# hedgepigdaniel/video-annotator

Hardware: AMD Instinct MI355X
Metric: stabilized frames/sec at 4K NV12, 1/2/4/8 GPU; remap % HBM roofline (higher is better)
Workload: dtype u8 pixels / f32 map / f64 rotations

## Files before the change

### video-annotator_amd/csrc/vstab_testhooks.cpp

```cpp
#include <algorithm>

#include "vstab_detect_host.hpp"
#include "vstab_hostlogic.hpp"
#include "vstab_pipeline.hpp"
#include "vstab_track_host.hpp"
#include "vstab_warp_bands.hpp"
#include "vstab_warp_request.hpp"

using namespace vstab;

extern "C" {
__attribute__((visibility("default"))) int vstabx_parse_records(const uint32_t *rec, int n, uint32_t seq, int expect_n, float *xy, unsigned char *status,
                                                                 int *n_out, int *next) {
    std::vector<float> pts;
    std::vector<uint8_t> st;
    int nx = 0;
    const LkParse r = lk_parse_records(rec, 0, n, seq, (size_t)expect_n, pts, st, &nx);
    for (size_t i = 0; i < st.size(); i++) xy[2 * i] = pts[2 * i], xy[2 * i + 1] = pts[2 * i + 1], status[i] = st[i];
    *n_out = (int)st.size(), *next = nx;
    return (int)r;
}
__attribute__((visibility("default"))) int vstabx_dmabuf_cache_sim(const unsigned long long *ids, const size_t *sizes, int n, int cap, long window,
                                                                    long long fail_id, long *counts, unsigned long long *bases) {
    DmaBufCache<unsigned long long> cache;
// ... 176 lines not shown
                                                                       double k, int block, int response, unsigned int cap, unsigned int canary,
                                                                       unsigned long long *keys_out, unsigned int *counts_out, unsigned int *tile_counts,
                                                                       int *max_bits_out, void *stream) {
    if (response != VSTAB_CORNER_MIN_EIGENVAL && response != VSTAB_CORNER_HARRIS) return fail(VSTAB_ERR_INVALID, "vstabx_corners_fused_block: response is 0 or 1");
    return corners_fused_hook("vstabx_corners_fused_block", gray, pitch, w, h, mask, pitch_mask, mask != nullptr, quality, cap, canary, keys_out, counts_out, tile_counts,
                              stream, response == VSTAB_CORNER_HARRIS, k, max_bits_out, block);
}
__attribute__((visibility("default"))) int vstabx_corners_fused_grad(const void *gray, size_t pitch, int w, int h, const void *mask, size_t pitch_mask, double quality,
                                                                      double k, int block, int gradient, int response, unsigned int cap, unsigned int canary,
                                                                      unsigned long long *keys_out, unsigned int *counts_out, unsigned int *tile_counts,
                                                                      int *max_bits_out, void *stream) {
    if (response != VSTAB_CORNER_MIN_EIGENVAL && response != VSTAB_CORNER_HARRIS) return fail(VSTAB_ERR_INVALID, "vstabx_corners_fused_grad: response is 0 or 1");
    return corners_fused_hook("vstabx_corners_fused_grad", gray, pitch, w, h, mask, pitch_mask, mask != nullptr, quality, cap, canary, keys_out, counts_out, tile_counts,
                              stream, response == VSTAB_CORNER_HARRIS, k, max_bits_out, block, gradient);
}

__attribute__((visibility("default"))) int vstabx_weighted_bands(int dw, int dh, int rwb, int lds_kb, double tail_rounds, const uint32_t *cost, int n_cost,
                                                                  int *out) {
    if (!out || dw < 1 || dh < 1 || (rwb != 4 && rwb != 8) || lds_kb < 1 || !(tail_rounds >= 0.0) || n_cost < 0)
        return fail(VSTAB_ERR_INVALID, "vstabx_weighted_bands: bad argument");
    FusedArgs ta = {};
    ta.w.dw = dw, ta.w.dh = dh;
    const unsigned grid = cost ? weighted_bands(ta, rwb, lds_kb, tail_rounds, cost, n_cost) : tile_schedule(ta, rwb, lds_kb, tail_rounds);
    for (int k = 0; k < 9; k++) out[k] = ta.band_y[k];
    for (int k = 0; k < 8; k++) out[9 + k] = ta.split_y[k];
    out[17] = ta.tiles_x, out[18] = (int)grid;
    return VSTAB_OK;
}
__attribute__((visibility("default"))) int vstabx_band_costs(const float *params, int nan_behind, int sw, int sh, int dw, int dh, int ts, uint32_t *cost, int n_cost) {
    if (!params || !cost || sw < 1 || sh < 1 || dw < 1 || dh < 1 || (ts != 8 && ts != 16) || n_cost != (int)div_up((unsigned)dh, (unsigned)ts))
        return fail(VSTAB_ERR_INVALID, "vstabx_band_costs: bad argument");
    std::vector<uint32_t> c;
    band_costs(params, nan_behind != 0, sw, sh, dw, dh, ts, c);
    std::copy(c.begin(), c.end(), cost);
    return VSTAB_OK;
}
__attribute__((visibility("default"))) int vstabx_band_cache_run(const float *params, int n, int sw, int sh, int dw, int dh, int map_mode, int rwb, int lds_kb,
                                                                  double tail_rounds, int *out, long *counts) {
    if (!params || !out || !counts || n < 1 || sw < 1 || sh < 1 || dw < 1 || dh < 1 || (rwb != 4 && rwb != 8) || lds_kb < 1 || !(tail_rounds >= 0.0))
        return fail(VSTAB_ERR_INVALID, "vstabx_band_cache_run: bad argument");
    BandCache cache;
    for (int i = 0; i < n; i++) {
        FusedArgs ta = {};
        ta.w.sw = sw, ta.w.sh = sh, ta.w.dw = dw, ta.w.dh = dh;
        const unsigned grid = cache.schedule(ta, params + 17 * (size_t)i, map_mode, rwb, lds_kb, tail_rounds);
        int *o = out + 19 * (size_t)i;
        for (int k = 0; k < 9; k++) o[k] = ta.band_y[k];
        for (int k = 0; k < 8; k++) o[9 + k] = ta.split_y[k];
        o[17] = ta.tiles_x, o[18] = (int)grid;
    }
    counts[0] = cache.hits, counts[1] = cache.misses, counts[2] = (long)cache.entries.size();
    return VSTAB_OK;
}

__attribute__((visibility("default"))) int vstabx_warp_route(int map_mode, int lens, int rs, int resample, int border_entry, int border_mode, int out_format, int keep,
                                                              int qmap, int *out) {
    if (!out) return fail(VSTAB_ERR_INVALID, "vstabx_warp_route: bad argument");
    const WarpRoute r = warp_route(map_mode, lens, rs != 0, resample, border_entry, border_mode, out_format, keep != 0, qmap != 0);
    out[0] = r.family, out[1] = r.block, out[2] = r.mode;
    return VSTAB_OK;
}

__attribute__((visibility("default"))) int vstabx_select_corners(const unsigned long long *keys, unsigned int n, int w, int h, int max_corners, double min_distance,
                                                                  float *xy, int *count) {
    if ((n > 0 && !keys) || !xy || !count || w < 1 || h < 1 || !(min_distance >= 0.0))
        return fail(VSTAB_ERR_INVALID, "vstabx_select_corners: bad argument");
    for (unsigned int i = 0; i < n; i++)
        if ((keys[i] & 0xffffffffu) >= (uint64_t)w * (uint64_t)h) return fail(VSTAB_ERR_INVALID, "vstabx_select_corners: a key names a pixel outside the image");
    std::vector<unsigned long long> k(keys, keys + n);
    std::vector<float> out;
    select_corners(k.data(), n, w, h, max_corners, min_distance, out);
    std::copy(out.begin(), out.end(), xy);
    *count = (int)(out.size() / 2);
    return VSTAB_OK;
}

__attribute__((visibility("default"))) int vstabx_detector_counters(const vstab_handle *h, long *out) {
    if (!h || !out) return fail(VSTAB_ERR_INVALID, "vstabx_detector_counters: bad argument");
    out[0] = h->detector.spec_over_cap(), out[1] = h->detector.fused_overflows(), out[2] = (long)h->detector.key_capacity();
    return VSTAB_OK;
}

__attribute__((visibility("default"))) int vstabx_pack_pyr(const void *y, size_t pitch_y, const void *uv, size_t pitch_uv, int w, int h, void *ring, void *dst,
                                                            size_t dpitch, void *stream) {
    if (!pack_pyr_ok(y, pitch_y, uv, pitch_uv, w, h, ring, dst, dpitch)) return -1;
    return launch_pack_pyr(static_cast<const uint8_t *>(y), pitch_y, static_cast<const uint8_t *>(uv), pitch_uv, w, h, static_cast<uint8_t *>(ring),
                           static_cast<uint8_t *>(dst), dpitch, static_cast<hipStream_t>(stream));
}
__attribute__((visibility("default"))) int vstabx_launch_pack_pyr(const void *y, size_t pitch_y, const void *uv, size_t pitch_uv, int w, int h, void *ring, void *dst,
                                                                   size_t dpitch, void *stream) {
    return launch_pack_pyr(static_cast<const uint8_t *>(y), pitch_y, static_cast<const uint8_t *>(uv), pitch_uv, w, h, static_cast<uint8_t *>(ring),
                           static_cast<uint8_t *>(dst), dpitch, static_cast<hipStream_t>(stream));
}
__attribute__((visibility("default"))) int vstabx_pyr_down_check(size_t pitch_src, int w, int h, size_t pitch_mid, size_t pitch_dst, int two_levels) {
    return two_levels ? check_pyr_down_x2(pitch_src, w, h, pitch_mid, pitch_dst) : check_pyr_down(pitch_src, w, h, pitch_dst);
}
}
```

### video-annotator_amd/csrc/vstab_warp_args.hpp

```cpp
#pragma once
#include "vstab_device.hpp"
#include "vstab_internal.hpp"

namespace vstab {

struct WarpArgs {
    const uint8_t *y;
    const uint8_t *uv;
    uint8_t *dst;
    uint8_t *dst_uv;
    size_t pitch_y, pitch_uv, pitch_dst, pitch_dst_uv;
    int sw, sh, dw, dh;
    MapParams p;
};

struct FusedArgs {
    WarpArgs w;
    MapParams32 p32;
    int lds_capacity_px;
    int src_vec_ok;
    int dst_vec_ok;
    int tiles_x, tiles_y;
    const int2 *qmap;
    int qpitch;
    float rs_d[9];
    float rs_den;
    int band_y[9];
    int split_y[8];
#ifdef VSTAB_DEV
    unsigned long long *timing;
    int ablate;
    int lds_pad;
#endif
    ColourCoef col;
};

template <typename K>
__device__ __forceinline__ void fetch_tap(const WarpArgs &a, const K &k, int X, int Y, int &b, int &g, int &r) {
    if ((unsigned)X < (unsigned)a.sw && (unsigned)Y < (unsigned)a.sh) {
        const int yv = a.y[(size_t)Y * a.pitch_y + X];
        const uint16_t c = *reinterpret_cast<const uint16_t *>(a.uv + (size_t)(Y >> 1) * a.pitch_uv + (X & ~1));
        yuv_to_bgr(k, yv, chroma_term(k, c & 255, c >> 8), b, g, r);
    } else {
        b = g = r = 0;
    }
}
__device__ __forceinline__ void fetch_tap(const WarpArgs &a, int X, int Y, int &b, int &g, int &r) { fetch_tap(a, CvtColor8{}, X, Y, b, g, r); }

template <typename K>
__device__ __forceinline__ uint32_t gather_pixel(const WarpArgs &a, const K &k, int sx, int sy) {
    const int X = sx >> 5, Y = sy >> 5;
    const uint32_t fx = sx & 31, fy = sy & 31;
    const int w00 = (32 - fx) * (32 - fy), w01 = fx * (32 - fy), w10 = (32 - fx) * fy, w11 = fx * fy;
    int b0, g0, r0, b1, g1, r1, b2, g2, r2, b3, g3, r3;
    fetch_tap(a, k, X, Y, b0, g0, r0);
    fetch_tap(a, k, X + 1, Y, b1, g1, r1);
    fetch_tap(a, k, X, Y + 1, b2, g2, r2);
    fetch_tap(a, k, X + 1, Y + 1, b3, g3, r3);
    const uint32_t B = (uint32_t)(b0 * w00 + b1 * w01 + b2 * w10 + b3 * w11 + 512) >> 10;
    const uint32_t G = (uint32_t)(g0 * w00 + g1 * w01 + g2 * w10 + g3 * w11 + 512) >> 10;
    const uint32_t R = (uint32_t)(r0 * w00 + r1 * w01 + r2 * w10 + r3 * w11 + 512) >> 10;
    return B | (G << 8) | (R << 16);
}

__device__ __forceinline__ uint32_t load_u32_bytes(const uint8_t *p, int valid) {
    uint32_t v = 0;
    for (int i = 0; i < 4; i++)
        if (i < valid) v |= (uint32_t)p[i] << (8 * i);
    return v;
}

vstab_status launch_warp_fused(const WarpArgs &a, const float params[17], int map_mode, bool nv12_out, bool src_vec_ok, bool dst_vec_ok,
                               const void *qmap, int qpitch, const float *rot_bottom, hipStream_t st, const float *dist = nullptr);
vstab_status launch_warp_fused_colour(const WarpArgs &a, const float params[17], int map_mode, bool nv12_out, bool src_vec_ok, bool dst_vec_ok, const ColourCoef &col,
                                      hipStream_t st);
vstab_status launch_warp_fused10(const WarpArgs &a, const float params[17], int map_mode, int blend, const float *rot_bottom, bool p010_out, bool src_vec_ok,
                                 bool dst_vec_ok, hipStream_t st, const ColourCoef *col = nullptr);

vstab_status launch_warp_planar(const WarpArgs &a, const float params[17], int map_mode, int depth, int blend, bool src_vec_ok, bool dst_vec_ok,
                                const float *rot_bottom, hipStream_t st, const float *dist = nullptr);

}
```

### video-annotator_amd/csrc/vstab_warp_bands.hpp

```cpp
#pragma once
#include <array>
#include <cmath>
#include <cstdint>
#include <cstring>
#include <mutex>
#include <vector>

#include "vstab_warp_tile.hpp"

namespace vstab {

static inline unsigned weighted_bands(FusedArgs &ta, int rwb, int lds_kb, double tail_rounds, const uint32_t *cost, int n_cost) {
    const unsigned even_grid = tile_schedule(ta, rwb, lds_kb, tail_rounds);
    const WarpArgs &a = ta.w;
    const int th = 4 * rwb, ts = th / 2;
    const int half_rows = (int)div_up(a.dh, ts);
    if (!cost || n_cost != half_rows) return even_grid;
    uint64_t total = 0;
    for (int i = 0; i < half_rows; i++) total += cost[i];
    if (total == 0) return even_grid;
    const int slots = 32 * std::max(1, std::min(8, (int)(160 / lds_kb)));
    int h = 0;
    uint64_t prefix = 0;
    ta.band_y[0] = 0;
    for (int k = 1; k < 8; k++) {
        while (h < half_rows && 8 * (prefix + cost[h]) <= (uint64_t)k * total) prefix += cost[h++];
        ta.band_y[k] = std::min(a.dh, h * ts);
    }
    ta.band_y[8] = a.dh;
    int share = 0;
    for (int k = 0; k < 8; k++) {
        const int rows = ta.band_y[k + 1] - ta.band_y[k];
        const int tall_rows_max = rows / th;
        const int tail_tall_rows = (int)std::min<long>(tall_rows_max, std::lround(tail_rounds * slots / ta.tiles_x));
        const int tall_rows = tall_rows_max - tail_tall_rows;
        ta.split_y[k] = ta.band_y[k] + tall_rows * th;
        const int n = tall_rows * ta.tiles_x + (int)div_up(ta.band_y[k + 1] - ta.split_y[k], ts) * ta.tiles_x;
        share = std::max(share, n);
    }
    return 8u * (unsigned)share;
}

constexpr uint32_t BAND_COST_DEAD = 135, BAND_COST_LIVE = 220;
constexpr double BAND_COST_PER_BLOCK = 0.45;

static inline void band_costs(const float params[17], bool nan_behind, int sw, int sh, int dw, int dh, int ts, std::vector<uint32_t> &cost) {
    const int tiles_x = (int)div_up(dw, 64), half_rows = (int)div_up(dh, ts);
    const double icx = params[0], icy = params[1], ifx = params[2], ify = params[3], ocx = params[4], ocy = params[5], ofx = params[6], ofy = params[7];
    const float *r = params + 8;
    std::vector<double> X((size_t)(tiles_x + 1) * 2), Y((size_t)(tiles_x + 1) * 2);
    auto corners = [&](int row, double *xo, double *yo) {
        const double vy = ((double)std::min(row * ts, dh - 1) - ocy) / ofy;
        for (int c = 0; c <= tiles_x; c++) {
            const double vx = ((double)std::min(c * 64, dw - 1) - ocx) / ofx;
            const double wx = r[0] * vx + r[1] * vy + r[2], wy = r[3] * vx + r[4] * vy + r[5], wz = r[6] * vx + r[7] * vy + r[8];
            if (!(wz > 0.0) && (nan_behind || wz == 0.0)) {
                xo[c] = yo[c] = NAN;
                continue;
            }
            const double ux = wx / wz, uy = wy / wz, rad = std::sqrt(ux * ux + uy * uy), k = rad > 0.0 ? std::atan(rad) / rad : 1.0;
            xo[c] = icx + ifx * ux * k, yo[c] = icy + ify * uy * k;
        }
    };
    cost.assign((size_t)half_rows, 0u);
    double *x0 = X.data(), *x1 = x0 + tiles_x + 1, *y0 = Y.data(), *y1 = y0 + tiles_x + 1;
    corners(0, x0, y0);
    for (int row = 0; row < half_rows; row++) {
        corners(row + 1, x1, y1);
        uint32_t sum = 0;
        for (int c = 0; c < tiles_x; c++) {
            const double xs[4] = {x0[c], x0[c + 1], x1[c], x1[c + 1]}, ys[4] = {y0[c], y0[c + 1], y1[c], y1[c + 1]};
            double mnx = xs[0], mxx = xs[0], mny = ys[0], mxy = ys[0];
            bool finite = true;
            for (int i = 0; i < 4; i++) {
                finite = finite && std::isfinite(xs[i]) && std::isfinite(ys[i]);
                mnx = std::min(mnx, xs[i]), mxx = std::max(mxx, xs[i]), mny = std::min(mny, ys[i]), mxy = std::max(mxy, ys[i]);
            }
            double blocks = 64.0 * ts * 4.0 / 16.0;
            if (finite) {
                if (mxx < -1.0 || mnx >= (double)sw || mxy < -1.0 || mny >= (double)sh) {
                    sum += BAND_COST_DEAD;
                    continue;
                }
                const double bw = std::min(mxx + 2.0, (double)sw) - std::max(mnx - 1.0, -1.0) + 8.0;
                const double bh = std::min(mxy + 2.0, (double)sh) - std::max(mny - 1.0, -1.0) + 2.0;
                blocks = std::max(bw, 8.0) * std::max(bh, 2.0) / 16.0;
            }
            sum += BAND_COST_LIVE + (uint32_t)std::min(blocks * BAND_COST_PER_BLOCK, 4096.0);
        }
        cost[(size_t)row] = sum;
        std::swap(x0, x1), std::swap(y0, y1);
    }
}

constexpr double BAND_CACHE_ANGLE = 1.5 * 3.14159265358979323846 / 180.0;
constexpr int BAND_CACHE_ENTRIES = 32;
struct BandCache {
    struct Entry {
        float fixed[8];
        int dims[8];
        float rot[9];
        int band_y[9], split_y[8];
        unsigned grid;
    };
    std::mutex mu;
    std::vector<Entry> entries;
    size_t next = 0;
    long hits = 0, misses = 0;

    unsigned schedule(FusedArgs &ta, const float params[17], int map_mode, int rwb, int lds_kb, double tail_rounds) {
        const WarpArgs &a = ta.w;
        const int dims[8] = {a.sw, a.sh, a.dw, a.dh, map_mode, rwb, lds_kb, (int)std::lround(tail_rounds * 64.0)};
        const double min_trace = 1.0 + 2.0 * std::cos(BAND_CACHE_ANGLE);
        std::lock_guard<std::mutex> lock(mu);
        for (const Entry &e : entries) {
            if (std::memcmp(e.fixed, params, sizeof e.fixed) || std::memcmp(e.dims, dims, sizeof dims)) continue;
            double tr = 0.0;
            for (int i = 0; i < 9; i++) tr += (double)e.rot[i] * params[8 + i];
            if (!(tr >= min_trace)) continue;
            tile_schedule(ta, rwb, lds_kb, tail_rounds);
            std::memcpy(ta.band_y, e.band_y, sizeof e.band_y), std::memcpy(ta.split_y, e.split_y, sizeof e.split_y);
            hits++;
            return e.grid;
        }
        misses++;
        std::vector<uint32_t> cost;
        band_costs(params, map_mode == MAP_FISH_TO_RECT, a.sw, a.sh, a.dw, a.dh, 2 * rwb, cost);
        Entry e;
        std::memcpy(e.fixed, params, sizeof e.fixed), std::memcpy(e.dims, dims, sizeof dims), std::memcpy(e.rot, params + 8, sizeof e.rot);
        e.grid = weighted_bands(ta, rwb, lds_kb, tail_rounds, cost.data(), (int)cost.size());
        std::memcpy(e.band_y, ta.band_y, sizeof e.band_y), std::memcpy(e.split_y, ta.split_y, sizeof e.split_y);
        if ((int)entries.size() < BAND_CACHE_ENTRIES) entries.push_back(e);
        else entries[next++ % BAND_CACHE_ENTRIES] = e;
        return e.grid;
    }
};

}
```

### video-annotator_amd/csrc/vstab_warp_fused.hip

```cpp
#include <algorithm>
#include <climits>
#include <cmath>
#include <cstddef>
#include <cstdlib>

#include "vstab_device10.hpp"
#include "vstab_warp_bands.hpp"
#include "vstab_warp_host.hpp"
#include "vstab_warp_tile.hpp"

namespace vstab {

template <int RW, int DEPTH, int BLEND>
__device__ __forceinline__ void sample_batched(const FusedArgs &ta, const int (&Xr)[RW], const int (&Yr)[RW], const int (&qxb)[RW], const int (&qyb)[RW],
                                               const uint32_t tile_lds, const uint32_t wb4, uint32_t (&out)[RW]) {
    constexpr bool PIX8 = DEPTH == 10 && BLEND == VSTAB_BLEND_FP16;
    constexpr int TG = RW < TAP_GROUP ? RW : TAP_GROUP;
    if constexpr (PIX8) {
#pragma unroll
        for (int j0 = 0; j0 < RW; j0 += TG) {
            uint2 t0[TG], t1[TG], t2[TG], t3[TG];
#pragma unroll
            for (int j = 0; j < TG; j++) {
                uint32_t ax8, au;
                asm("v_lshl_add_u32 %0, %1, 3, %2" : "=v"(ax8) : "v"(Xr[j0 + j]), "s"(tile_lds));
                asm("v_mad_u32_u24 %0, %1, %2, %3" : "=v"(au) : "v"(Yr[j0 + j]), "s"(wb4), "v"(ax8));
                const LdsPair *u = reinterpret_cast<const LdsPair *>(au), *l = reinterpret_cast<const LdsPair *>(au + wb4);
                const u32x2 v0 = u[0], v1 = u[1], v2 = l[0], v3 = l[1];
                t0[j] = make_uint2(v0.x, v0.y), t1[j] = make_uint2(v1.x, v1.y), t2[j] = make_uint2(v2.x, v2.y), t3[j] = make_uint2(v3.x, v3.y);
            }
#pragma unroll
            for (int j = 0; j < TG; j++) out[j0 + j] = blend_bgr10h(t0[j], t1[j], t2[j], t3[j], qxb[j0 + j] & 31, qyb[j0 + j] & 31);
        }
    } else
#pragma unroll
    for (int j0 = 0; j0 < RW; j0 += TG) {
        uint32_t t0[TG], t1[TG], t2[TG], t3[TG];
#pragma unroll
        for (int j = 0; j < TG; j++) {
            uint32_t ax4, au;
            asm("v_lshl_add_u32 %0, %1, 2, %2" : "=v"(ax4) : "v"(Xr[j0 + j]), "s"(tile_lds));
            asm("v_mad_u32_u24 %0, %1, %2, %3" : "=v"(au) : "v"(Yr[j0 + j]), "s"(wb4), "v"(ax4));
            const LdsWord *u = reinterpret_cast<const LdsWord *>(au), *l = reinterpret_cast<const LdsWord *>(au + wb4);
            t0[j] = u[0], t1[j] = u[1], t2[j] = l[0], t3[j] = l[1];
        }
#pragma unroll
        for (int j = 0; j < TG; j++) {
#ifdef VSTAB_DEV
            if (ta.ablate & 2) out[j0 + j] = t0[j] ^ t1[j] ^ t2[j] ^ t3[j] ^ (qxb[j0 + j] & 31) ^ (qyb[j0 + j] & 31);
            else
#endif
            out[j0 + j] = DEPTH == 10 ? blend_bgr10<BLEND>(t0[j], t1[j], t2[j], t3[j], qxb[j0 + j] & 31, qyb[j0 + j] & 31)
                                      : blend_bgrx(t0[j], t1[j], t2[j], t3[j], qxb[j0 + j] & 31, qyb[j0 + j] & 31);
// ... 371 lines not shown
            if (ta.dst_vec_ok) {
                const uint32_t lo = (uint32_t)__builtin_amdgcn_ds_bpermute(4 * p0, (int)out[j]);
                const uint32_t hi = (uint32_t)__builtin_amdgcn_ds_bpermute(4 * p0 + 4, (int)out[j]);
                const uint32_t d = __builtin_amdgcn_perm(hi, lo, sel);
                if (lane < nfull) *reinterpret_cast<uint32_t *>(o + (uint32_t)(4 * lane)) = d;
                else if (lane == nfull && rem) {
                    uint32_t l4 = 4u * (uint32_t)lane;
                    if constexpr (ModeTraits<BASE>::dist || COLOUR) asm volatile("" : "+v"(l4));
                    for (int i = 0; i < rem; i++) o[l4 + i] = (d >> (8 * i)) & 255;
                }
            } else if (col_live) {
                o[3 * lane] = out[j] & 255, o[3 * lane + 1] = (out[j] >> 8) & 255, o[3 * lane + 2] = (out[j] >> 16) & 255;
            }
        }
    } else {
        Coef kc = {};
        if constexpr (COLOUR) kc = colour_coef_here();
#pragma unroll
        for (int j = 0; j < RW; j++) {
            const int y = y0 + wave * RW + j;
            if (y >= a.dh) break;
            const uint32_t yb = bgr_to_y(kc, out[j]);
            const uint32_t y1 = (uint32_t)__builtin_amdgcn_mov_dpp((int)yb, 0x55, 0xf, 0xf, true);
            const uint32_t y2 = (uint32_t)__builtin_amdgcn_mov_dpp((int)yb, 0xaa, 0xf, 0xf, true);
            const uint32_t y3 = (uint32_t)__builtin_amdgcn_mov_dpp((int)yb, 0xff, 0xf, 0xf, true);
            const uint32_t yw = yb | (y1 << 8) | (y2 << 16) | (y3 << 24);
            uint8_t *o = a.dst + ((size_t)(uint32_t)y * a.pitch_dst + (uint32_t)x);
            if (!(lane & 3) && col_live) {
                if (ta.dst_vec_ok && x + 4 <= a.dw) {
                    *reinterpret_cast<uint32_t *>(o) = yw;
                } else {
                    for (int i = 0; i < 4 && x + i < a.dw; i++) o[i] = (yw >> (8 * i)) & 255;
                }
            }
            if (!(y & 1)) {
                const uint32_t cb = bgr_to_uv(kc, out[j]);
                const uint32_t c2 = (uint32_t)__builtin_amdgcn_mov_dpp((int)cb, 0xaa, 0xf, 0xf, true);
                const uint32_t cw = cb | (c2 << 16);
                uint8_t *c = a.dst_uv + ((size_t)(uint32_t)(y >> 1) * a.pitch_dst_uv + (uint32_t)x);
                if (!(lane & 3) && col_live) {
                    if (ta.dst_vec_ok && x + 2 < a.dw) {
                        *reinterpret_cast<uint32_t *>(c) = cw;
                    } else {
                        for (int i = 0; i < 4 && x + (i & ~1) < a.dw; i++) c[i] = (cw >> (8 * i)) & 255;
                    }
                }
            }
        }
    }
    VSTAB_STAMP(7);
    return true;
}

template <int RWB, int MODE, int FMT, bool CACHED, int DEPTH = 8, int BLEND = 0, bool COLOUR = false>
__global__ void __launch_bounds__(256, DEPTH == 10 ? 5 : (RWB == 8 || map_mode_is_rs(MODE)) ? VSTAB_WARP_WAVES - 1 : VSTAB_WARP_WAVES) k_warp_fused(FusedArgs ta) {
    extern __shared__ __attribute__((aligned(16))) uint32_t smem[];
    constexpr int TH = 4 * RWB, TS = TH / 2;
    if (VSTAB_WARP_PRIO) __builtin_amdgcn_s_setprio(VSTAB_WARP_PRIO);
    const int k = (int)(blockIdx.x & 7u);
    const int y_lo = ta.band_y[k], y_sp = ta.split_y[k], y_hi = ta.band_y[k + 1];
    const int n_tall = ((y_sp - y_lo) / TH) * ta.tiles_x;
    const int idx = (int)(blockIdx.x >> 3);
    int x0, ys, n_half;
    if (idx < n_tall) {
        const int row = idx / ta.tiles_x;
        x0 = (idx - row * ta.tiles_x) * 64, ys = y_lo + row * TH;
        n_half = warp_tile<RWB, RWB, MODE, FMT, CACHED, true, DEPTH, BLEND, COLOUR>(ta, smem, x0, ys) ? 0 : 2;
    } else {
        const int i2 = idx - n_tall, row = i2 / ta.tiles_x;
        x0 = (i2 - row * ta.tiles_x) * 64, ys = y_sp + row * TS, n_half = 1;
        if (ys >= y_hi) return;
    }
#pragma unroll 1
    for (int i = 0; i < n_half; i++) warp_tile<RWB, RWB / 2, MODE, FMT, CACHED, false, DEPTH, BLEND, COLOUR>(ta, smem, x0, ys + i * TS);
}

}

using namespace vstab;

namespace vstab {
#ifdef VSTAB_DEV
static unsigned long long *g_dev_timing = nullptr;
extern "C" __attribute__((visibility("default"))) void vstab_dev_set_timing(void *p) { g_dev_timing = static_cast<unsigned long long *>(p); }
#endif

vstab_status launch_warp_fused10(const WarpArgs &a, const float params[17], int map_mode, int blend, const float *rot_bottom, bool p010_out, bool src_vec_ok,
                                 bool dst_vec_ok, hipStream_t st, const ColourCoef *col) {
    FusedArgs ta;
    fill_fused_args(ta, a, params, src_vec_ok, dst_vec_ok, nullptr, 0, rot_bottom);
    if (col) ta.col = *col;
    const int lds_kb = 40;
    const bool half = blend == VSTAB_BLEND_FP16;
    const int rwb = 8;
    const long tiles = (long)div_up(a.dw, 64) * div_up(a.dh, 4 * rwb);
    const dim3 grid(tile_schedule(ta, rwb, lds_kb, tiles > 1024 ? 0.5 : 0.0));
    if (half) ta.lds_capacity_px /= 2;
    const size_t lds_bytes = (size_t)lds_kb * 1024;
    vstab_status status = VSTAB_OK;
    with_map_mode(map_mode, rot_bottom != nullptr, [&](auto mode) {
        with_either<VSTAB_BLEND_FP16, VSTAB_BLEND_EXACT>(half, [&](auto blend_c) {
            with_either<3, 2>(p010_out, [&](auto fmt) {
                with_bool(col != nullptr, [&](auto colour) {
                    constexpr int MODE = decltype(mode)::value;
                    if constexpr (map_mode_fish_to_pinhole(map_mode_base(MODE)))
                        launch_kernel(k_warp_fused<8, MODE, decltype(fmt)::value, false, 10, decltype(blend_c)::value, decltype(colour)::value>, grid, dim3(256),
                                      lds_bytes, st, ta);
                    else
                        status = fail(VSTAB_ERR_INVALID, "launch_warp_fused10: the 10-bit tiled kernels serve map modes 0, 1 and 5 only");
                });
            });
        });
    });
    if (status != VSTAB_OK) return status;
    VSTAB_HIP_TRY(hipGetLastError());
    return VSTAB_OK;
}

struct FusedShape {
    int rwb;
    size_t lds_bytes;
    unsigned grid;
};
static FusedShape fused_shape(FusedArgs &ta, const float params[17], int map_mode, bool per_frame_ideal) {
    const WarpArgs &a = ta.w;
    const long tiles32 = (long)div_up(a.dw, 64) * div_up(a.dh, 32);
    int rwb = tiles32 < 1536 ? 4 : 8, lds_kb = rwb == 4 ? 20 : 40;
    double tail_rounds = (double)div_up(a.dw, 64) * div_up(a.dh, 4 * rwb) > 256.0 * (160 / lds_kb) ? 0.5 : 0.0;
#ifdef VSTAB_DEV
    if (const char *e = getenv("VSTAB_ROWS")) rwb = atoi(e) == 4 ? 4 : 8;
    if (const char *e = getenv("VSTAB_LDS_KB")) lds_kb = atoi(e);
    if (const char *e = getenv("VSTAB_TAIL_ROUNDS")) tail_rounds = atof(e);
#endif
    bool weighted = tail_rounds > 0.0 && per_frame_ideal &&
                    (map_mode == MAP_CREATEMAP_CL || map_mode == MAP_FISH_TO_RECT || map_mode == MAP_CREATEMAP_CL_OPENCL);
#ifdef VSTAB_DEV
    if (const char *e = getenv("VSTAB_BANDS")) weighted = weighted && atoi(e) != 0;
#endif
    static BandCache band_cache;
    const unsigned grid = weighted ? band_cache.schedule(ta, params, map_mode, rwb, lds_kb, tail_rounds) : tile_schedule(ta, rwb, lds_kb, tail_rounds);
    return {rwb, (size_t)lds_kb * 1024, grid};
}

vstab_status launch_warp_fused(const WarpArgs &a, const float params[17], int map_mode, bool nv12_out, bool src_vec_ok, bool dst_vec_ok,
                               const void *qmap, int qpitch, const float *rot_bottom, hipStream_t st, const float *dist) {
    FusedArgs ta;
    fill_fused_args(ta, a, params, src_vec_ok, dst_vec_ok, qmap, qpitch, rot_bottom, dist);
#ifdef VSTAB_DEV
    ta.timing = g_dev_timing;
    static const int ablate = getenv("VSTAB_ABLATE") ? atoi(getenv("VSTAB_ABLATE")) : 0;
    ta.ablate = ablate;
    ta.lds_pad = getenv("VSTAB_LDS_PAD") ? atoi(getenv("VSTAB_LDS_PAD")) & ~3 : 0;
#endif
    const FusedShape shape = fused_shape(ta, params, map_mode, !dist && !qmap && !rot_bottom);
    const int rwb = shape.rwb;
    const size_t lds_bytes = shape.lds_bytes;
    const dim3 grid(shape.grid);
    if (dist) {
        if (nv12_out || qmap || rot_bottom) return fail(VSTAB_ERR_INVALID, "launch_warp_fused: the distorted-lens kernels emit BGR8 from one rotation per frame");
        with_dist_mode(map_mode, [&](auto mode) {
            with_either<8, 4>(rwb == 8, [&](auto rows) {
                launch_kernel(k_warp_fused<decltype(rows)::value, decltype(mode)::value, 0, false>, grid, dim3(256), lds_bytes, st, ta);
            });
        });
        VSTAB_HIP_TRY(hipGetLastError());
        return VSTAB_OK;
    }
    with_map_mode(qmap ? (int)VSTAB_MAP_CREATEMAP_CL : map_mode, !qmap && rot_bottom != nullptr, [&](auto mode) {
        with_bool(qmap != nullptr, [&](auto cached) {
            with_either<8, 4>(rwb == 8, [&](auto rows) {
                with_either<1, 0>(nv12_out, [&](auto fmt) {
                    constexpr int MODE = decltype(mode)::value;
                    constexpr bool CACHED = decltype(cached)::value;
                    if constexpr (!CACHED || MODE == MAP_CREATEMAP_CL)
                        launch_kernel(k_warp_fused<decltype(rows)::value, MODE, decltype(fmt)::value, CACHED>, grid, dim3(256), lds_bytes, st, ta);
                });
            });
        });
    });
    VSTAB_HIP_TRY(hipGetLastError());
    return VSTAB_OK;
}


vstab_status launch_warp_fused_colour(const WarpArgs &a, const float params[17], int map_mode, bool nv12_out, bool src_vec_ok, bool dst_vec_ok, const ColourCoef &col,
                                      hipStream_t st) {
    FusedArgs ta;
    fill_fused_args(ta, a, params, src_vec_ok, dst_vec_ok, nullptr, 0, nullptr);
    ta.col = col;
    const FusedShape shape = fused_shape(ta, params, map_mode, true);
    with_map_mode(map_mode, [&](auto mode) {
        with_either<8, 4>(shape.rwb == 8, [&](auto rows) {
            with_either<1, 0>(nv12_out, [&](auto fmt) {
                launch_kernel(k_warp_fused<decltype(rows)::value, decltype(mode)::value, decltype(fmt)::value, false, 8, 0, true>, dim3(shape.grid), dim3(256),
                              shape.lds_bytes, st, ta);
            });
        });
    });
    VSTAB_HIP_TRY(hipGetLastError());
    return VSTAB_OK;
}

vstab_status preload_fused_kernels() {
    hipFuncAttributes at;
    VSTAB_HIP_TRY(hipFuncGetAttributes(&at, reinterpret_cast<const void *>((&k_warp_fused<8, MAP_CREATEMAP_CL_OPENCL, 0, false, 8, 0>))));
    return VSTAB_OK;
}

}
```

### video-annotator_amd/csrc/vstab_warp_host.hpp

```cpp
#pragma once
#include <hip/hip_ext.h>

#include <type_traits>

#include "vstab_internal.hpp"
#include "vstab_resample.hpp"
#include "vstab_warp_request.hpp"

namespace vstab {

inline bool ptr_aligned(const void *p, size_t a) { return (reinterpret_cast<uintptr_t>(p) % a) == 0; }

inline MapParams map_params(const float params[17]) {
    MapParams m;
    m.icx = params[0], m.icy = params[1], m.ifx = params[2], m.ify = params[3];
    m.ocx = params[4], m.ocy = params[5], m.ofx = params[6], m.ofy = params[7];
    for (int i = 0; i < 9; i++) m.r[i] = params[8 + i];
    return m;
}
inline MapParams32 map_params32(const float params[17], const float *dist = nullptr) {
    MapParams32 m = {params[0] * 32.0f, params[1] * 32.0f, params[2] * 32.0f, params[3] * 32.0f, params[10], params[13], params[16], {0.0f, 0.0f, 0.0f, 0.0f}};
    if (dist) m.d = {dist[0], dist[1], dist[2], dist[3]};
    return m;
}
inline void fill_warp_args(WarpArgs &a, const void *y, size_t pitch_y, const void *uv, size_t pitch_uv, int sw, int sh, const float params[17], void *dst,
                           size_t pitch_dst, void *dst_uv, size_t pitch_dst_uv, int dw, int dh) {
    a.y = (const uint8_t *)y, a.uv = (const uint8_t *)uv, a.dst = (uint8_t *)dst, a.dst_uv = (uint8_t *)dst_uv;
    a.pitch_y = pitch_y, a.pitch_uv = pitch_uv, a.pitch_dst = pitch_dst, a.pitch_dst_uv = pitch_dst_uv;
    a.sw = sw, a.sh = sh, a.dw = dw, a.dh = dh;
    a.p = map_params(params);
}
template <typename Args>
void fill_rolling_shutter(Args &a, const float params[17], const float *rot_bottom, int dh) {
    for (int k = 0; k < 9; k++) a.rs_d[k] = rot_bottom ? rot_bottom[k] - params[8 + k] : 0.0f;
    a.rs_den = (float)(dh > 1 ? dh - 1 : 1);
}
inline void fill_fused_args(FusedArgs &ta, const WarpArgs &a, const float params[17], bool src_vec_ok, bool dst_vec_ok, const void *qmap, int qpitch,
                            const float *rot_bottom, const float *dist = nullptr) {
    ta.w = a;
    ta.p32 = map_params32(params, dist);
    ta.src_vec_ok = src_vec_ok, ta.dst_vec_ok = dst_vec_ok;
    ta.qmap = static_cast<const int2 *>(qmap), ta.qpitch = qpitch;
    fill_rolling_shutter(ta, params, rot_bottom, a.dh);
#ifdef VSTAB_DEV
    ta.timing = nullptr, ta.ablate = 0, ta.lds_pad = 0;
#endif
    ta.col = ColourCoef{};
}

struct StagedOffsets32 {
    bool rows, chroma;
};
inline StagedOffsets32 staged_offsets32(size_t pitch_y, size_t pitch_uv, int sh) {
    const bool rows = pitch_y < (1u << 24) && pitch_uv < (1u << 24) && (uint64_t)pitch_y * sh < (1ull << 32);
    return {rows, rows && (uint64_t)pitch_uv * (sh / 2) < (1ull << 32)};
}

template <int M>
using mode_constant = std::integral_constant<int, M>;
template <typename F>
void with_map_mode(int map_mode, F &&f) {
    switch (map_mode) {
        case VSTAB_MAP_CREATEMAP_CL: f(mode_constant<MAP_CREATEMAP_CL>{}); break;
        case VSTAB_MAP_FISH_TO_RECT: f(mode_constant<MAP_FISH_TO_RECT>{}); break;
        case VSTAB_MAP_FISH_TO_FISH: f(mode_constant<MAP_FISH_TO_FISH>{}); break;
        case VSTAB_MAP_RECT_TO_RECT: f(mode_constant<MAP_RECT_TO_RECT>{}); break;
        case VSTAB_MAP_RECT_TO_FISH: f(mode_constant<MAP_RECT_TO_FISH>{}); break;
        default: f(mode_constant<MAP_CREATEMAP_CL_OPENCL>{}); break;
    }
}
template <typename F>
void with_map_mode(int map_mode, bool rs, F &&f) {
    if (!rs) return with_map_mode(map_mode, f);
    switch (map_mode) {
        case VSTAB_MAP_CREATEMAP_CL: f(mode_constant<MAP_RS_CREATEMAP_CL>{}); break;
        case VSTAB_MAP_CREATEMAP_CL_OPENCL: f(mode_constant<MAP_RS_CREATEMAP_CL_OPENCL>{}); break;
        default: f(mode_constant<MAP_RS_FISH_TO_RECT>{}); break;
    }
}
template <typename F>
void with_dist_mode(int map_mode, F &&f) {
    if (map_mode == VSTAB_MAP_FISH_TO_RECT) f(mode_constant<MAP_FISHD_TO_RECT>{});
    else f(mode_constant<MAP_FISHD_TO_FISH>{});
}
template <typename F>
void with_kernel_mode(int mode, F &&f) {
    switch (mode) {
        case MAP_CREATEMAP_CL: f(mode_constant<MAP_CREATEMAP_CL>{}); break;
        case MAP_FISH_TO_RECT: f(mode_constant<MAP_FISH_TO_RECT>{}); break;
        case MAP_FISH_TO_FISH: f(mode_constant<MAP_FISH_TO_FISH>{}); break;
        case MAP_RECT_TO_RECT: f(mode_constant<MAP_RECT_TO_RECT>{}); break;
        case MAP_RECT_TO_FISH: f(mode_constant<MAP_RECT_TO_FISH>{}); break;
        case MAP_CREATEMAP_CL_OPENCL: f(mode_constant<MAP_CREATEMAP_CL_OPENCL>{}); break;
        case MAP_RS_CREATEMAP_CL: f(mode_constant<MAP_RS_CREATEMAP_CL>{}); break;
        case MAP_RS_FISH_TO_RECT: f(mode_constant<MAP_RS_FISH_TO_RECT>{}); break;
        case MAP_RS_CREATEMAP_CL_OPENCL: f(mode_constant<MAP_RS_CREATEMAP_CL_OPENCL>{}); break;
        case MAP_FISHD_TO_RECT: f(mode_constant<MAP_FISHD_TO_RECT>{}); break;
        case MAP_FISHD_TO_FISH: f(mode_constant<MAP_FISHD_TO_FISH>{}); break;
        case MAP_RS_FISHD_TO_RECT: f(mode_constant<MAP_RS_FISHD_TO_RECT>{}); break;
        case MAP_RECTD_TO_RECT: f(mode_constant<MAP_RECTD_TO_RECT>{}); break;
// ... 161 lines not shown
```

Baseline: 32160.

## Schedule fused warp tiles through a per-frame device tile table balancing dead tiles

```diff
diff --git a/video-annotator_amd/csrc/vstab_testhooks.cpp b/video-annotator_amd/csrc/vstab_testhooks.cpp
--- a/video-annotator_amd/csrc/vstab_testhooks.cpp
+++ b/video-annotator_amd/csrc/vstab_testhooks.cpp
@@ -252,6 +252,37 @@
     counts[0] = cache.hits, counts[1] = cache.misses, counts[2] = (long)cache.entries.size();
     return VSTAB_OK;
 }
+__attribute__((visibility("default"))) int vstabx_tile_table(const float *params, int n, int sw, int sh, int dw, int dh, int map_mode, int rwb, int lds_kb,
+                                                              double tail_rounds, int *out, uint32_t *table, int cap, uint32_t *tile_cost, long *counts) {
+    if (!params || !out || !table || !counts || n < 1 || cap < 1 || sw < 1 || sh < 1 || dw < 1 || dh < 1 || (rwb != 4 && rwb != 8) || lds_kb < 1 || !(tail_rounds >= 0.0))
+        return fail(VSTAB_ERR_INVALID, "vstabx_tile_table: bad argument");
+    BandCache cache;
+    const size_t n_tiles = (size_t)div_up((unsigned)dh, 2u * rwb) * div_up((unsigned)dw, 64u);
+    for (int i = 0; i < n; i++) {
+        FusedArgs ta = {};
+        ta.w.sw = sw, ta.w.sh = sh, ta.w.dw = dw, ta.w.dh = dh;
+        const float *p = params + 17 * (size_t)i;
+        const BandCache::Entry &e = cache.entries[(size_t)cache.find(ta, p, map_mode, rwb, lds_kb, tail_rounds, 0)];
+        if (e.table.size() > (size_t)cap) return fail(VSTAB_ERR_INVALID, "vstabx_tile_table: cap is smaller than the grid");
+        int *o = out + 19 * (size_t)i;
+        for (int k = 0; k < 9; k++) o[k] = ta.band_y[k];
+        for (int k = 0; k < 8; k++) o[9 + k] = ta.split_y[k];
+        o[17] = ta.tiles_x, o[18] = (int)e.grid;
+        std::copy(e.table.begin(), e.table.end(), table + (size_t)cap * i);
+        if (tile_cost) {
+            std::vector<uint32_t> rows, tiles;
+            band_costs(p, map_mode == MAP_FISH_TO_RECT, sw, sh, dw, dh, 2 * rwb, rows, &tiles);
+            std::copy(tiles.begin(), tiles.end(), tile_cost + n_tiles * i);
+        }
+    }
+    counts[0] = cache.hits, counts[1] = cache.misses, counts[2] = (long)cache.entries.size();
+    return VSTAB_OK;
+}
+__attribute__((visibility("default"))) int vstabx_fused_force(int tile32, int table) {
+    if (tile32 < -1 || tile32 > 1 || table < -1 || table > 1) return fail(VSTAB_ERR_INVALID, "vstabx_fused_force: -1, 0 or 1");
+    fused_force(tile32, table);
+    return VSTAB_OK;
+}
 
 __attribute__((visibility("default"))) int vstabx_warp_route(int map_mode, int lens, int rs, int resample, int border_entry, int border_mode, int out_format, int keep,
                                                               int qmap, int *out) {
diff --git a/video-annotator_amd/csrc/vstab_warp_args.hpp b/video-annotator_amd/csrc/vstab_warp_args.hpp
--- a/video-annotator_amd/csrc/vstab_warp_args.hpp
+++ b/video-annotator_amd/csrc/vstab_warp_args.hpp
@@ -33,7 +33,12 @@
     int lds_pad;
 #endif
     ColourCoef col;
+    const uint32_t *tile_table;
 };
+
+constexpr uint32_t TILE_NONE = 0xffffffffu;
+constexpr int TILE_COL_BITS = 12, TILE_ROW_BITS = 19;
+constexpr uint32_t tile_entry(int col, int half_row, bool tall) { return (uint32_t)col | (uint32_t)half_row << TILE_COL_BITS | (tall ? 1u << 31 : 0u); }
 
 template <typename K>
 __device__ __forceinline__ void fetch_tap(const WarpArgs &a, const K &k, int X, int Y, int &b, int &g, int &r) {
@@ -74,6 +79,7 @@
                                const void *qmap, int qpitch, const float *rot_bottom, hipStream_t st, const float *dist = nullptr);
 vstab_status launch_warp_fused_colour(const WarpArgs &a, const float params[17], int map_mode, bool nv12_out, bool src_vec_ok, bool dst_vec_ok, const ColourCoef &col,
                                       hipStream_t st);
+void fused_force(int tile32, int table);
 vstab_status launch_warp_fused10(const WarpArgs &a, const float params[17], int map_mode, int blend, const float *rot_bottom, bool p010_out, bool src_vec_ok,
                                  bool dst_vec_ok, hipStream_t st, const ColourCoef *col = nullptr);
 
diff --git a/video-annotator_amd/csrc/vstab_warp_bands.hpp b/video-annotator_amd/csrc/vstab_warp_bands.hpp
--- a/video-annotator_amd/csrc/vstab_warp_bands.hpp
+++ b/video-annotator_amd/csrc/vstab_warp_bands.hpp
@@ -10,7 +10,8 @@
 
 namespace vstab {
 
-static inline unsigned weighted_bands(FusedArgs &ta, int rwb, int lds_kb, double tail_rounds, const uint32_t *cost, int n_cost) {
+static inline unsigned weighted_bands(FusedArgs &ta, int rwb, int lds_kb, double tail_rounds, const uint32_t *cost, int n_cost,
+                                      const uint64_t *target8 = nullptr) {
     const unsigned even_grid = tile_schedule(ta, rwb, lds_kb, tail_rounds);
     const WarpArgs &a = ta.w;
     const int th = 4 * rwb, ts = th / 2;
@@ -24,7 +25,8 @@
     uint64_t prefix = 0;
     ta.band_y[0] = 0;
     for (int k = 1; k < 8; k++) {
-        while (h < half_rows && 8 * (prefix + cost[h]) <= (uint64_t)k * total) prefix += cost[h++];
+        const uint64_t aim = target8 ? target8[k] : (uint64_t)k * total;
+        while (h < half_rows && 8 * (prefix + cost[h]) <= aim) prefix += cost[h++];
         ta.band_y[k] = std::min(a.dh, h * ts);
     }
     ta.band_y[8] = a.dh;
@@ -44,7 +46,8 @@
 constexpr uint32_t BAND_COST_DEAD = 135, BAND_COST_LIVE = 220;
 constexpr double BAND_COST_PER_BLOCK = 0.45;
 
-static inline void band_costs(const float params[17], bool nan_behind, int sw, int sh, int dw, int dh, int ts, std::vector<uint32_t> &cost) {
+static inline void band_costs(const float params[17], bool nan_behind, int sw, int sh, int dw, int dh, int ts, std::vector<uint32_t> &cost,
+                              std::vector<uint32_t> *tile_cost = nullptr) {
     const int tiles_x = (int)div_up(dw, 64), half_rows = (int)div_up(dh, ts);
     const double icx = params[0], icy = params[1], ifx = params[2], ify = params[3], ocx = params[4], ocy = params[5], ofx = params[6], ofy = params[7];
     const float *r = params + 8;
@@ -63,6 +66,7 @@
         }
     };
     cost.assign((size_t)half_rows, 0u);
+    if (tile_cost) tile_cost->assign((size_t)half_rows * tiles_x, 0u);
     double *x0 = X.data(), *x1 = x0 + tiles_x + 1, *y0 = Y.data(), *y1 = y0 + tiles_x + 1;
     corners(0, x0, y0);
     for (int row = 0; row < half_rows; row++) {
@@ -80,21 +84,107 @@
             if (finite) {
                 if (mxx < -1.0 || mnx >= (double)sw || mxy < -1.0 || mny >= (double)sh) {
                     sum += BAND_COST_DEAD;
+                    if (tile_cost) (*tile_cost)[(size_t)row * tiles_x + c] = BAND_COST_DEAD;
                     continue;
                 }
                 const double bw = std::min(mxx + 2.0, (double)sw) - std::max(mnx - 1.0, -1.0) + 8.0;
                 const double bh = std::min(mxy + 2.0, (double)sh) - std::max(mny - 1.0, -1.0) + 2.0;
                 blocks = std::max(bw, 8.0) * std::max(bh, 2.0) / 16.0;
             }
-            sum += BAND_COST_LIVE + (uint32_t)std::min(blocks * BAND_COST_PER_BLOCK, 4096.0);
+            const uint32_t live = BAND_COST_LIVE + (uint32_t)std::min(blocks * BAND_COST_PER_BLOCK, 4096.0);
+            sum += live;
+            if (tile_cost) (*tile_cost)[(size_t)row * tiles_x + c] = live;
         }
         cost[(size_t)row] = sum;
         std::swap(x0, x1), std::swap(y0, y1);
     }
 }
 
+struct TileOrder {
+    std::vector<uint32_t> table;
+    unsigned grid = 0;
+    int n_live[8] = {}, n_dead[8] = {};
+    uint64_t cost[8] = {};
+};
+static inline void tile_order(FusedArgs &ta, int rwb, int lds_kb, double tail_rounds, const uint32_t *tile_cost, TileOrder &o) {
+    const WarpArgs &a = ta.w;
+    const int th = 4 * rwb, ts = th / 2, tiles_x = (int)div_up(a.dw, 64), half_rows = (int)div_up(a.dh, ts);
+    auto cost_at = [&](int r, int c) { return tile_cost[(size_t)r * tiles_x + c]; };
+    auto dead = [&](int r, int c) { return cost_at(r, c) == BAND_COST_DEAD; };
+    std::vector<uint32_t> row_live((size_t)half_rows, 0u);
+    uint64_t total = 0;
+    for (int r = 0; r < half_rows; r++)
+        for (int c = 0; c < tiles_x; c++) {
+            total += cost_at(r, c);
+            if (!dead(r, c)) row_live[(size_t)r] += cost_at(r, c);
+        }
+    struct Item {
+        uint32_t entry, cost;
+    };
+    std::vector<Item> live[8], pool;
+    std::vector<int> owner;
+    size_t n[8];
+    uint64_t target8[8] = {};
+    int prev_band[9], prev_split[8];
+    for (int pass = 0; pass < 3; pass++) {
+        weighted_bands(ta, rwb, lds_kb, tail_rounds, row_live.data(), half_rows, pass ? target8 : nullptr);
+        if (pass && !std::memcmp(prev_band, ta.band_y, sizeof prev_band) && !std::memcmp(prev_split, ta.split_y, sizeof prev_split)) break;
+        std::memcpy(prev_band, ta.band_y, sizeof prev_band), std::memcpy(prev_split, ta.split_y, sizeof prev_split);
+        pool.clear();
+        for (int k = 0; k < 8; k++) {
+            live[k].clear();
+            if (ta.band_y[k] == ta.band_y[k + 1]) continue;
+            for (int y = ta.band_y[k]; y < ta.split_y[k]; y += th) {
+                const int r = y / ts;
+                for (int c = 0; c < tiles_x; c++)
+                    (dead(r, c) && dead(r + 1, c) ? pool : live[k]).push_back({tile_entry(c, r, true), cost_at(r, c) + cost_at(r + 1, c)});
+            }
+            const int r0 = ta.split_y[k] / ts, r1 = (int)div_up(ta.band_y[k + 1], ts);
+            for (int r = r0; r < r1; r++)
+                for (int c = 0; c < tiles_x; c++)
+                    if (!dead(r, c)) live[k].push_back({tile_entry(c, r, false), cost_at(r, c)});
+            for (int r = r0; r < r1; r += 2) {
+                const bool two = r + 1 < r1, fits = two && (r + 2) * ts <= a.dh;
+                for (int c = 0; c < tiles_x; c++) {
+                    if (fits && dead(r, c) && dead(r + 1, c)) {
+                        pool.push_back({tile_entry(c, r, true), 2 * BAND_COST_DEAD});
+                        continue;
+                    }
+                    if (dead(r, c)) pool.push_back({tile_entry(c, r, false), BAND_COST_DEAD});
+                    if (two && dead(r + 1, c)) pool.push_back({tile_entry(c, r + 1, false), BAND_COST_DEAD});
+                }
+            }
+        }
+        uint64_t dealt[8] = {};
+        for (int k = 0; k < 8; k++) {
+            n[k] = live[k].size(), o.cost[k] = 0;
+            for (const Item &it : live[k]) o.cost[k] += it.cost;
+            o.n_live[k] = (int)n[k];
+        }
+        owner.assign(pool.size(), 0);
+        for (size_t i = 0; i < pool.size(); i++) {
+            int best = 0;
+            for (int k = 1; k < 8; k++)
+                if (n[k] < n[best] || (n[k] == n[best] && o.cost[k] < o.cost[best])) best = k;
+            owner[i] = best, n[best]++, o.cost[best] += pool[i].cost, dealt[best] += pool[i].cost;
+        }
+        if (pool.empty()) break;
+        uint64_t aim = 0;
+        for (int k = 0; k < 8; k++) target8[k] = aim, aim += total > 8 * dealt[k] ? total - 8 * dealt[k] : 0;
+    }
+    size_t longest = 0;
+    for (int k = 0; k < 8; k++) longest = std::max(longest, n[k]), o.n_dead[k] = (int)n[k] - o.n_live[k];
+    o.grid = 8u * (unsigned)longest;
+    o.table.assign((size_t)o.grid, TILE_NONE);
+    size_t pos[8] = {};
+    for (int k = 0; k < 8; k++)
+        for (const Item &it : live[k]) o.table[8 * pos[k]++ + (size_t)k] = it.entry;
+    for (size_t i = 0; i < pool.size(); i++) o.table[8 * pos[owner[i]]++ + (size_t)owner[i]] = pool[i].entry;
+}
+
 constexpr double BAND_CACHE_ANGLE = 1.5 * 3.14159265358979323846 / 180.0;
 constexpr int BAND_CACHE_ENTRIES = 32;
+constexpr size_t TILE_SLOT_ENTRIES = 32768;
 struct BandCache {
     struct Entry {
         float fixed[8];
@@ -102,37 +192,110 @@
         float rot[9];
         int band_y[9], split_y[8];
         unsigned grid;
+        int device = -1;
+        std::vector<uint32_t> table;
+        bool resident = false;
+        hipStream_t up_stream = nullptr;
+    };
+    struct Slab {
+        int device;
+        uint32_t *dev, *host;
+        hipEvent_t uploaded[BAND_CACHE_ENTRIES];
+        bool handed_out[BAND_CACHE_ENTRIES];
     };
     std::mutex mu;
     std::vector<Entry> entries;
+    std::vector<Slab> slabs;
     size_t next = 0;
     long hits = 0, misses = 0;
 
     unsigned schedule(FusedArgs &ta, const float params[17], int map_mode, int rwb, int lds_kb, double tail_rounds) {
+        std::lock_guard<std::mutex> lock(mu);
+        return entries[(size_t)find(ta, params, map_mode, rwb, lds_kb, tail_rounds, -1)].grid;
+    }
+
+    int find(FusedArgs &ta, const float params[17], int map_mode, int rwb, int lds_kb, double tail_rounds, int device) {
         const WarpArgs &a = ta.w;
         const int dims[8] = {a.sw, a.sh, a.dw, a.dh, map_mode, rwb, lds_kb, (int)std::lround(tail_rounds * 64.0)};
         const double min_trace = 1.0 + 2.0 * std::cos(BAND_CACHE_ANGLE);
-        std::lock_guard<std::mutex> lock(mu);
-        for (const Entry &e : entries) {
-            if (std::memcmp(e.fixed, params, sizeof e.fixed) || std::memcmp(e.dims, dims, sizeof dims)) continue;
+        for (size_t i = 0; i < entries.size(); i++) {
+            const Entry &e = entries[i];
+            if (e.device != device || std::memcmp(e.fixed, params, sizeof e.fixed) || std::memcmp(e.dims, dims, sizeof dims)) continue;
             double tr = 0.0;
-            for (int i = 0; i < 9; i++) tr += (double)e.rot[i] * params[8 + i];
+            for (int k = 0; k < 9; k++) tr += (double)e.rot[k] * params[8 + k];
             if (!(tr >= min_trace)) continue;
             tile_schedule(ta, rwb, lds_kb, tail_rounds);
             std::memcpy(ta.band_y, e.band_y, sizeof e.band_y), std::memcpy(ta.split_y, e.split_y, sizeof e.split_y);
             hits++;
-            return e.grid;
+            return (int)i;
         }
         misses++;
-        std::vector<uint32_t> cost;
-        band_costs(params, map_mode == MAP_FISH_TO_RECT, a.sw, a.sh, a.dw, a.dh, 2 * rwb, cost);
+        std::vector<uint32_t> cost, tile_cost;
+        band_costs(params, map_mode == MAP_FISH_TO_RECT, a.sw, a.sh, a.dw, a.dh, 2 * rwb, cost, device >= 0 ? &tile_cost : nullptr);
         Entry e;
         std::memcpy(e.fixed, params, sizeof e.fixed), std::memcpy(e.dims, dims, sizeof dims), std::memcpy(e.rot, params + 8, sizeof e.rot);
-        e.grid = weighted_bands(ta, rwb, lds_kb, tail_rounds, cost.data(), (int)cost.size());
+        e.device = device;
+        if (device >= 0) {
+            TileOrder o;
+            tile_order(ta, rwb, lds_kb, tail_rounds, tile_cost.data(), o);
+            e.grid = o.grid, e.table.swap(o.table);
+        } else {
+            e.grid = weighted_bands(ta, rwb, lds_kb, tail_rounds, cost.data(), (int)cost.size());
+        }
         std::memcpy(e.band_y, ta.band_y, sizeof e.band_y), std::memcpy(e.split_y, ta.split_y, sizeof e.split_y);
-        if ((int)entries.size() < BAND_CACHE_ENTRIES) entries.push_back(e);
-        else entries[next++ % BAND_CACHE_ENTRIES] = e;
-        return e.grid;
+        if ((int)entries.size() < BAND_CACHE_ENTRIES) {
+            entries.push_back(std::move(e));
+            return (int)entries.size() - 1;
+        }
+        const size_t slot = next++ % BAND_CACHE_ENTRIES;
+        entries[slot] = std::move(e);
+        return (int)slot;
+    }
+
+    Slab *slab_of(int device) {
+        for (Slab &s : slabs)
+            if (s.device == device) return &s;
+        Slab s = {};
+        s.device = device;
+        const size_t bytes = BAND_CACHE_ENTRIES * TILE_SLOT_ENTRIES * sizeof(uint32_t);
+        if (hipMalloc((void **)&s.dev, bytes) != hipSuccess || hipHostMalloc((void **)&s.host, bytes, hipHostMallocDefault) != hipSuccess) {
+            (void)hipGetLastError();
+            if (s.dev) (void)hipFree(s.dev);
+            return nullptr;
+        }
+        for (int i = 0; i < BAND_CACHE_ENTRIES; i++)
+            if (hipEventCreateWithFlags(&s.uploaded[i], hipEventDisableTiming) != hipSuccess) {
+                (void)hipGetLastError();
+                return nullptr;
+            }
+        slabs.push_back(s);
+        return &slabs.back();
+    }
+
+    const uint32_t *acquire(int slot, hipStream_t st) {
+        Entry &e = entries[(size_t)slot];
+        if (e.device < 0 || e.table.empty() || e.table.size() > TILE_SLOT_ENTRIES) return nullptr;
+        Slab *s = slab_of(e.device);
+        if (!s) return nullptr;
+        uint32_t *dev = s->dev + (size_t)slot * TILE_SLOT_ENTRIES, *host = s->host + (size_t)slot * TILE_SLOT_ENTRIES;
+        bool ok = true;
+        if (!e.resident) {
+            if (s->handed_out[slot]) ok = hipDeviceSynchronize() == hipSuccess, s->handed_out[slot] = !ok;
+            if (ok) {
+                std::memcpy(host, e.table.data(), e.table.size() * sizeof(uint32_t));
+                ok = hipMemcpyAsync(dev, host, e.table.size() * sizeof(uint32_t), hipMemcpyHostToDevice, st) == hipSuccess &&
+                     hipEventRecord(s->uploaded[slot], st) == hipSuccess;
+            }
+            e.resident = ok, e.up_stream = st;
+        } else if (e.up_stream != st) {
+            ok = hipStreamWaitEvent(st, s->uploaded[slot], 0) == hipSuccess;
+        }
+        if (!ok) {
+            (void)hipGetLastError();
+            return nullptr;
+        }
+        s->handed_out[slot] = true;
+        return dev;
     }
 };
 
diff --git a/video-annotator_amd/csrc/vstab_warp_fused.hip b/video-annotator_amd/csrc/vstab_warp_fused.hip
--- a/video-annotator_amd/csrc/vstab_warp_fused.hip
+++ b/video-annotator_amd/csrc/vstab_warp_fused.hip
@@ -1,4 +1,5 @@
 #include <algorithm>
+#include <atomic>
 #include <climits>
 #include <cmath>
 #include <cstddef>
@@ -476,11 +477,37 @@
     return true;
 }
 
+constexpr bool tile_table_kernel(int rwb, int mode, bool cached, int depth, bool colour) {
+    return rwb == 8 && depth == 8 && !cached && !colour && (mode == MAP_CREATEMAP_CL || mode == MAP_CREATEMAP_CL_OPENCL || mode == MAP_FISH_TO_RECT);
+}
 template <int RWB, int MODE, int FMT, bool CACHED, int DEPTH = 8, int BLEND = 0, bool COLOUR = false>
 __global__ void __launch_bounds__(256, DEPTH == 10 ? 5 : (RWB == 8 || map_mode_is_rs(MODE)) ? VSTAB_WARP_WAVES - 1 : VSTAB_WARP_WAVES) k_warp_fused(FusedArgs ta) {
     extern __shared__ __attribute__((aligned(16))) uint32_t smem[];
     constexpr int TH = 4 * RWB, TS = TH / 2;
     if (VSTAB_WARP_PRIO) __builtin_amdgcn_s_setprio(VSTAB_WARP_PRIO);
+    if constexpr (tile_table_kernel(RWB, MODE, CACHED, DEPTH, COLOUR)) {
+        int x0, ys;
+        bool tall;
+        if (ta.tile_table) {
+            typedef const __attribute__((address_space(4))) uint32_t *ConstWords;
+            const uint32_t e = reinterpret_cast<ConstWords>(reinterpret_cast<uintptr_t>(ta.tile_table))[blockIdx.x];
+            if (e == TILE_NONE) return;
+            x0 = (int)(e & ((1u << TILE_COL_BITS) - 1u)) * 64, ys = (int)((e >> TILE_COL_BITS) & ((1u << TILE_ROW_BITS) - 1u)) * TS, tall = (e >> 31) != 0;
+        } else {
+            const int kb = (int)(blockIdx.x & 7u), ib = (int)(blockIdx.x >> 3);
+            const int b_lo = ta.band_y[kb], b_sp = ta.split_y[kb], b_hi = ta.band_y[kb + 1];
+            const int b_tall = ((b_sp - b_lo) / TH) * ta.tiles_x;
+            tall = ib < b_tall;
+            const int i2 = tall ? ib : ib - b_tall, row = i2 / ta.tiles_x;
+            x0 = (i2 - row * ta.tiles_x) * 64, ys = tall ? b_lo + row * TH : b_sp + row * TS;
+            if (!tall && ys >= b_hi) return;
+        }
+        int halves = 1;
+        if (tall) halves = warp_tile<RWB, RWB, MODE, FMT, CACHED, true, DEPTH, BLEND, COLOUR>(ta, smem, x0, ys) ? 0 : 2;
+#pragma unroll 1
+        for (int i = 0; i < halves; i++) warp_tile<RWB, RWB / 2, MODE, FMT, CACHED, false, DEPTH, BLEND, COLOUR>(ta, smem, x0, ys + i * TS);
+        return;
+    }
     const int k = (int)(blockIdx.x & 7u);
     const int y_lo = ta.band_y[k], y_sp = ta.split_y[k], y_hi = ta.band_y[k + 1];
     const int n_tall = ((y_sp - y_lo) / TH) * ta.tiles_x;
@@ -541,29 +568,56 @@
     return VSTAB_OK;
 }
 
+static BandCache g_band_cache;
+static std::atomic<int> g_force_tile32{-1}, g_force_table{-1};
+void fused_force(int tile32, int table) { g_force_tile32 = tile32, g_force_table = table; }
 struct FusedShape {
     int rwb;
     size_t lds_bytes;
     unsigned grid;
+    std::unique_lock<std::mutex> lock;
+    int slot = -1;
+    void used(hipStream_t st) {
+        if (slot >= 0) lock.unlock();
+    }
 };
-static FusedShape fused_shape(FusedArgs &ta, const float params[17], int map_mode, bool per_frame_ideal) {
+static FusedShape fused_shape(FusedArgs &ta, const float params[17], int map_mode, bool per_frame_ideal, const hipStream_t *table_st = nullptr) {
     const WarpArgs &a = ta.w;
     const long tiles32 = (long)div_up(a.dw, 64) * div_up(a.dh, 32);
     int rwb = tiles32 < 1536 ? 4 : 8, lds_kb = rwb == 4 ? 20 : 40;
+    const int force_tile32 = g_force_tile32, force_table = g_force_table;
+    if (force_tile32 >= 0) rwb = force_tile32 ? 8 : 4, lds_kb = rwb == 4 ? 20 : 40;
     double tail_rounds = (double)div_up(a.dw, 64) * div_up(a.dh, 4 * rwb) > 256.0 * (160 / lds_kb) ? 0.5 : 0.0;
 #ifdef VSTAB_DEV
     if (const char *e = getenv("VSTAB_ROWS")) rwb = atoi(e) == 4 ? 4 : 8;
     if (const char *e = getenv("VSTAB_LDS_KB")) lds_kb = atoi(e);
     if (const char *e = getenv("VSTAB_TAIL_ROUNDS")) tail_rounds = atof(e);
 #endif
-    bool weighted = tail_rounds > 0.0 && per_frame_ideal &&
-                    (map_mode == MAP_CREATEMAP_CL || map_mode == MAP_FISH_TO_RECT || map_mode == MAP_CREATEMAP_CL_OPENCL);
+    const bool dead_mode = per_frame_ideal && (map_mode == MAP_CREATEMAP_CL || map_mode == MAP_FISH_TO_RECT || map_mode == MAP_CREATEMAP_CL_OPENCL);
+    bool weighted = tail_rounds > 0.0 && dead_mode;
+    bool table = (force_table < 0 ? weighted : force_table != 0 && dead_mode) && rwb == 8 && table_st != nullptr;
 #ifdef VSTAB_DEV
     if (const char *e = getenv("VSTAB_BANDS")) weighted = weighted && atoi(e) != 0;
-#endif
-    static BandCache band_cache;
-    const unsigned grid = weighted ? band_cache.schedule(ta, params, map_mode, rwb, lds_kb, tail_rounds) : tile_schedule(ta, rwb, lds_kb, tail_rounds);
-    return {rwb, (size_t)lds_kb * 1024, grid};
+    if (const char *e = getenv("VSTAB_TILE_TABLE")) table = table && atoi(e) != 0;
+#endif
+    FusedShape shape = {rwb, (size_t)lds_kb * 1024, 0u, {}, -1};
+    int device = -1;
+    hipStreamCaptureStatus capture = hipStreamCaptureStatusNone;
+    if (table && (hipStreamIsCapturing(*table_st, &capture) != hipSuccess || capture != hipStreamCaptureStatusNone || hipGetDevice(&device) != hipSuccess)) {
+        (void)hipGetLastError();
+        table = false;
+    }
+    if (table) {
+        shape.lock = std::unique_lock<std::mutex>(g_band_cache.mu);
+        const int slot = g_band_cache.find(ta, params, map_mode, rwb, lds_kb, tail_rounds, device);
+        if ((ta.tile_table = g_band_cache.acquire(slot, *table_st))) {
+            shape.grid = g_band_cache.entries[(size_t)slot].grid, shape.slot = slot;
+            return shape;
+        }
+        shape.lock.unlock();
+    }
+    shape.grid = weighted ? g_band_cache.schedule(ta, params, map_mode, rwb, lds_kb, tail_rounds) : tile_schedule(ta, rwb, lds_kb, tail_rounds);
+    return shape;
 }
 
 vstab_status launch_warp_fused(const WarpArgs &a, const float params[17], int map_mode, bool nv12_out, bool src_vec_ok, bool dst_vec_ok,
@@ -576,7 +630,7 @@
     ta.ablate = ablate;
     ta.lds_pad = getenv("VSTAB_LDS_PAD") ? atoi(getenv("VSTAB_LDS_PAD")) & ~3 : 0;
 #endif
-    const FusedShape shape = fused_shape(ta, params, map_mode, !dist && !qmap && !rot_bottom);
+    FusedShape shape = fused_shape(ta, params, map_mode, !dist && !qmap && !rot_bottom, &st);
     const int rwb = shape.rwb;
     const size_t lds_bytes = shape.lds_bytes;
     const dim3 grid(shape.grid);
@@ -602,6 +656,7 @@
             });
         });
     });
+    shape.used(st);
     VSTAB_HIP_TRY(hipGetLastError());
     return VSTAB_OK;
 }
diff --git a/video-annotator_amd/csrc/vstab_warp_host.hpp b/video-annotator_amd/csrc/vstab_warp_host.hpp
--- a/video-annotator_amd/csrc/vstab_warp_host.hpp
+++ b/video-annotator_amd/csrc/vstab_warp_host.hpp
@@ -46,6 +46,7 @@
     ta.timing = nullptr, ta.ablate = 0, ta.lds_pad = 0;
 #endif
     ta.col = ColourCoef{};
+    ta.tile_table = nullptr;
 }
 
 struct StagedOffsets32 {
```

Measured after the change: 30890. -3.9%, worse.
